# 3dlg-hcvc/minsu3d

Hardware: AMD Instinct MI355X
Metric: scenes/sec (fwd+bwd) PointGroup on ~150k-pt 2cm voxels (higher is better)
Workload: dtype f32; 1 GPU; PointGroup m=16, synthetic ScanNet-shaped scenes (~144k points, ~106k voxels @2cm each), 4 scenes/GPU/step, grouping+ScoreNet branch on, fwd+loss+bwd+Adam; scenes_per_gpu=4, parallelism=dp1, grouping_inputs=GT labels, GT offsets + N(0,4cm) (random-init net groups nothing)

## Files before the change

### include/minsu3d_hip.h

```cpp
#ifndef MINSU3D_HIP_H
#define MINSU3D_HIP_H
#include <stddef.h>
#include <stdint.h>

#ifdef __cplusplus
extern "C" {
#endif

#define MS3D_E_WORKSPACE 10001
#define MS3D_E_UNSUPPORTED 10002
#define MS3D_E_INTERNAL 10003

typedef void *ms3d_stream_t;

const char *ms3d_version(void);

size_t ms3d_ballquery_workspace_bytes(int n);
int ms3d_ballquery_batch_p(int n, int meanActive, float radius, const float *xyz, const uint8_t *batch_idxs,
                           const int *batch_offsets, int n_scenes, int max_scene_points, int *idx,
                           int *start_len, int *n_active , int *capped ,
                           void *workspace, size_t workspace_bytes, ms3d_stream_t stream);

size_t ms3d_bfs_workspace_bytes(int N);
int ms3d_pg_bfs_cluster(const int16_t *semantic_label, const int *ball_query_idxs, long n_edges ,
// ... 310 lines not shown
                                 void *ev_wg_stop, float *ws_wgrad, ms3d_stream_t wgrad_stream, int join,
                                 float *wgrad_slabs, int *wgrad_deferred_nblk, void *wgrad_deferred_launch, int precision,
                                 ms3d_stream_t stream);
int ms3d_spconv_wgrad_is_bf16x3_g(int Vout, int K, int Cin, int Cout, int offset_list, int submanifold);
int ms3d_spconv_backward_weight_g(const float *in, const float *dout, const int *nbr, int Vin, int Vout, int K, int Cin,
                                  int Cout, float *dW, const float *pre_scale, const float *pre_shift, int pre_relu,
                                  float *partial_ws, const int *ol_kt_start, const int *ol_entries, int submanifold,
                                  int precision, ms3d_stream_t stream);
int ms3d_spconv_layer_backward_g(const float *x, const float *dy, const float *wf_buf, const int *nbr_fwd,
                                 const int *nbr_bwd, int Vin, int Vout, int K, int Cin, int Cout, const float *scale,
                                 const float *shift, const float *mean, const float *invstd, int pre_relu, int training,
                                 int need_dx, float *dx, const float *dx_add, float *dgb, float *dW, float *ws,
                                 const int *ol_fwd_kt_start, const int *ol_fwd_entries, const int *pl_bwd_tile_start,
                                 const int *pl_bwd_entries, void *ev_start, void *ev_stop, void *ev_wg_start,
                                 void *ev_wg_stop, float *ws_wgrad, ms3d_stream_t wgrad_stream, int join,
                                 float *wgrad_slabs, int *wgrad_deferred_nblk, void *wgrad_deferred_launch, int precision,
                                 int submanifold, ms3d_stream_t stream);
size_t ms3d_spconv_wgrad_launch_bytes(void);
int ms3d_spconv_wgrad_is_table_walk(int Vout, int K, int Cin, int Cout, int offset_list);
int ms3d_spconv_wgrad_multi(const void *descs, int n_desc, int total_blocks, int variant, ms3d_stream_t stream);
int ms3d_wgrad_reduce_blocks(long n, const float *slabs, const float *dW, int *wide );
int ms3d_wgrad_reduce_multi(const void *descs, int n_desc, int total_blocks, ms3d_stream_t stream);

int ms3d_bn_stats(const float *x, long V, int C, float eps, float momentum, const float *gamma, const float *beta,
                  float *running_mean, float *running_var, float *mean, float *invstd, float *scale, float *shift,
                  float *partial_ws, int partial_rows, ms3d_stream_t stream);
int ms3d_bn_apply(const float *x, long V, int C, const float *scale, const float *shift, int relu, float *y,
                  ms3d_stream_t stream);
int ms3d_reduce_partials(const float *partial, int nparts, int n, float *out, ms3d_stream_t stream);
int ms3d_column_sum(const float *x, long V, int C, float *partial_ws, int partial_rows, float *out2c, ms3d_stream_t stream);
int ms3d_bn_bwd_apply(const float *dz, const float *x, long V, int C, const float *scale, const float *mean,
                      const float *invstd, const float *s1s2, float *dx, ms3d_stream_t stream);
int ms3d_bn_bwd_reduce_apply(const float *partial, int nparts, const float *dz, const float *x, long V, int C,
                             const float *scale, const float *mean, const float *invstd, const float *add, float *dx,
                             float *s1s2, ms3d_stream_t stream);
int ms3d_bn_bwd_apply_add(const float *dz, const float *x, long V, int C, const float *scale, const float *mean,
                          const float *invstd, const float *s1s2, const float *add, float *dx, ms3d_stream_t stream);
int ms3d_bn_bwd_partial(const float *dy, const float *x, long V, int C, const float *scale, const float *shift,
                        const float *mean, const float *invstd, int relu, float *dz, float *partial_ws,
                        int partial_rows, int *nparts_out , ms3d_stream_t stream);

int ms3d_dense_tile_cells(void);
int ms3d_dense_tile_channels(void);
int ms3d_dense_cell_map(const int *coords, int V, const int *origin , int divisor, int B, int X, int Y, int Z,
                        int *cell_row, int *row_cell, int *counts_dev, int *counts , ms3d_stream_t stream);
int ms3d_dense_scatter(const float *F, long n_rows, long ld, const int *cell_row, const int *row_index, int B, int C, int X,
                       int Y, int Z, float *out , ms3d_stream_t stream);
int ms3d_dense_gather(const float *grid, int B, int C, int X, int Y, int Z, const int *cells, long n, float *out,
                      ms3d_stream_t stream);
size_t ms3d_dense_occupancy_workspace_bytes(void);
int ms3d_dense_occupancy(const float *grid, int B, int C, int X, int Y, int Z, unsigned char *keep, int *rank,
                         int *n_kept , void *workspace, size_t workspace_bytes, ms3d_stream_t stream);
int ms3d_dense_cells_emit(const unsigned char *keep, const int *rank, int B, int X, int Y, int Z, int *out_coords,
                          int *out_cells, ms3d_stream_t stream);

int ms3d_proposal_cross_intersection(const int *pair_point, const int *pair_cluster, int S, int P, int *inter ,
                                     ms3d_stream_t stream);
int ms3d_nms_greedy(const int *inter, const int *order, int P, float threshold, unsigned char *suppressed_ws, int *pick,
                    int *n_pick, ms3d_stream_t stream);

int ms3d_elastic_distort(const double *xyz , int N, float *noise, float *noise_tmp, int bx, int by, int bz,
                         double gran, double mag, double *out , ms3d_stream_t stream);

int ms3d_adam_chunk_elems(void);
int ms3d_adam_step(const int *chunks, int n_chunks, void *const *p_ptrs, const void *const *g_ptrs, void *const *m_ptrs,
                   void *const *v_ptrs, const long *sizes, float lr, float beta1, float beta2, float eps,
                   float weight_decay, double bias_correction1, double bias_correction2, ms3d_stream_t stream);
int ms3d_adam_step_multi(const int *chunks, int n_chunks, void *const *p_ptrs, const void *const *g_ptrs,
                         void *const *m_ptrs, void *const *v_ptrs, const long *sizes, const float *coef, float beta1,
                         float beta2, float eps, float weight_decay, ms3d_stream_t stream);

size_t ms3d_scan_i32_workspace_bytes(void);
int ms3d_scan_i32(const int *in, int *out, int n, int *total_out_dev, void *workspace, ms3d_stream_t stream);

int ms3d_point_losses_blocks(long N);
int ms3d_point_losses_forward(const float *scores , const short *labels , const float *pred_offsets ,
                              const float *centre , const float *xyz , const short *instance_ids ,
                              long N, int C, float *d_scores, float *d_norm, float *d_dir, double *partial_ws, float *out5,
                              ms3d_stream_t stream);
int ms3d_point_losses_scale_grads(float *d_scores, long n_scores, float *d_norm, const float *d_dir, long n_off,
                                  const float *out5, const float *g_sem, const float *g_norm, const float *g_dir,
                                  ms3d_stream_t stream);

#ifdef __cplusplus
}
#endif
#endif
```

### minsu3d_amd/_lib.py

```python
import ctypes as C
import os

_HERE = os.path.dirname(os.path.abspath(__file__))
LIB_PATH = os.environ.get("MS3D_LIB") or os.path.join(_HERE, "lib", "libminsu3d_hip.so")
_lib = None


class HipLibraryError(RuntimeError):
    pass


def lib():
    global _lib
    if _lib is None:
        if not os.path.exists(LIB_PATH):
            raise HipLibraryError(
                f"{LIB_PATH} is missing: run `python -c 'import __graft_entry__ as g; g.build()'` "
                "(hipcc --offload-arch=gfx950). There is no CPU fallback in the product path.")
        _lib = C.CDLL(LIB_PATH)
        _lib.ms3d_version.restype = C.c_char_p
        for name in ("ms3d_ballquery_workspace_bytes", "ms3d_bfs_workspace_bytes", "ms3d_hais_workspace_bytes",
                     "ms3d_coord_workspace_bytes", "ms3d_coords_expand_workspace_bytes",
                     "ms3d_coords_union_workspace_bytes", "ms3d_broadcast_reduce_workspace_bytes",
                     "ms3d_chconv_wgrad_ws_floats", "ms3d_kattn_dbias_ws_floats", "ms3d_inorm_workspace_bytes",
                     "ms3d_dense_occupancy_workspace_bytes", "ms3d_kmap_pairs_workspace_bytes",
                     "ms3d_qattn_ws_floats", "ms3d_qattn_backward_ws_floats", "ms3d_vattn_backward_kv_ws_floats"):
            if hasattr(_lib, name):
                getattr(_lib, name).restype = C.c_size_t
        if hasattr(_lib, "ms3d_qattn_chunks"):
            _lib.ms3d_qattn_chunks.restype = C.c_long
    return _lib


E_UNSUPPORTED = 10002


def check(rc, what):
    if rc != 0:
        raise HipLibraryError(f"{what} failed with code {rc}")


def ptr(t):
    if t is None:
        return C.c_void_p(0)
    assert t.is_contiguous(), "tensor must be contiguous"
    return C.c_void_p(t.data_ptr())


_raw_stream = None


def stream_handle():
    global _raw_stream
    import torch
    if _raw_stream is None:
        _raw_stream = getattr(torch._C, "_cuda_getCurrentRawStream", False)
    if _raw_stream:
        return C.c_void_p(_raw_stream(torch._C._cuda_getDevice()))
    return C.c_void_p(torch.cuda.current_stream().cuda_stream)
```

### minsu3d_amd/backend.py

```python
import ctypes as C
import os
import weakref

import numpy as np
import torch

from . import _lib

_BACKEND = None


def get_backend():
    global _BACKEND
    if _BACKEND is None:
        _BACKEND = HipBackend()
    return _BACKEND


def set_backend(b):
    global _BACKEND
    prev = _BACKEND
    _BACKEND = b
    return prev

# ... 212 lines not shown

    def __init__(self):
        self.lib = _lib.lib()
        self.ext = _load_host_ext() if not os.environ.get("MS3D_LIB") else None
        self.ws = _Workspace()
        self.kernel_timer = None
        self.weight_token = 0
        self.matmul_precision_aware = True
        self._prep_table = None

    @staticmethod
    def _dev(t):
        if not t.is_cuda:
            if not torch.cuda.is_available():
                raise _lib.HipLibraryError("HipBackend needs a GPU (got a CPU tensor and no device is present); "
                                           "the product path has no CPU fallback")
            t = t.cuda(non_blocking=True)
        return t.contiguous()

    def ballquery_batch_p(self, coords, batch_idxs, batch_offsets, radius, meanActive, max_scene_points=0):
        coords = self._dev(coords); batch_idxs = self._dev(batch_idxs); batch_offsets = self._dev(batch_offsets)
        n = coords.size(0)
        dev = coords.device
        start_len = torch.zeros((n, 2), dtype=torch.int32, device=dev)
        if n == 0:
            return torch.zeros(0, dtype=torch.int32, device=dev), start_len
        if max_scene_points <= 0:
            max_scene_points = SCENE_BOUNDS.get(batch_offsets)
            if max_scene_points is None:
                max_scene_points = int((batch_offsets[1:] - batch_offsets[:-1]).max().item())
                SCENE_BOUNDS.put(batch_offsets, max_scene_points)
        ws_bytes = self.lib.ms3d_ballquery_workspace_bytes(n)
        ws = self.ws.get("bq", ws_bytes, dev)
        n_active, capped = C.c_int(0), C.c_int(0)
        timer = self.kernel_timer
        ev0 = timer.op_begin() if timer is not None else None
        hint_key = (round(float(radius), 6), int(meanActive))
        hints = self.__dict__.setdefault("_bq_mean_active", {})
        meanActive = max(int(meanActive), hints.get(hint_key, 0))
        while True:
            idx = torch.empty(n * meanActive, dtype=torch.int32, device=dev)
            rc = self.lib.ms3d_ballquery_batch_p(
                n, int(meanActive), C.c_float(radius), _lib.ptr(coords), _lib.ptr(batch_idxs),
                _lib.ptr(batch_offsets), int(batch_offsets.numel() - 1), int(max_scene_points), _lib.ptr(idx),
                _lib.ptr(start_len), C.byref(n_active), C.byref(capped), _lib.ptr(ws), C.c_size_t(ws.numel()),
                _lib.stream_handle())
            _lib.check(rc, "ms3d_ballquery_batch_p")
            if n_active.value <= n * meanActive:
                break
            meanActive = int(n_active.value // n + 1)
            hints[hint_key] = meanActive + meanActive // 8 + 1
        if ev0 is not None:
            timer.op_end("ballquery_batch_p", ev0, n * 20 + n_active.value * (6.64 * 12 + 4))
        GRAPHS.put(start_len, int(capped.value))
        return idx[:n_active.value], start_len

    def _bfs(self, fn_name, args_head, ball_idx, start_len, args_tail):
        hint = int(GRAPHS.get(start_len, -1))
        ball_idx = self._dev(ball_idx); start_len = self._dev(start_len)
        N = start_len.size(0)
        dev = start_len.device
        cluster_idxs = torch.empty((max(N, 1), 2), dtype=torch.int32, device=dev)
        cluster_offsets = torch.empty(N + 1, dtype=torch.int32, device=dev)
        ws_bytes = self.lib.ms3d_bfs_workspace_bytes(N)
        ws = self.ws.get("bfs", ws_bytes, dev)
        counts = (C.c_int * 2)(0, 0)
        args_tail = tuple(hint if a is _HINT else a for a in args_tail)
        timer = self.kernel_timer
        ev0 = timer.op_begin() if timer is not None else None
        rc = getattr(self.lib, fn_name)(*args_head, _lib.ptr(ball_idx), C.c_long(ball_idx.numel()), _lib.ptr(start_len), N,
                                        *args_tail,
                                        _lib.ptr(cluster_idxs), _lib.ptr(cluster_offsets), counts, _lib.ptr(ws),
                                        C.c_size_t(ws.numel()), _lib.stream_handle())
        _lib.check(rc, fn_name)
        if ev0 is not None:
            timer.op_end(fn_name[5:], ev0, ball_idx.numel() * 4 + N * 14 + counts[1] * 8)
        return cluster_idxs[:counts[1]], cluster_offsets[:counts[0] + 1]

    def pg_bfs_cluster(self, semantic_label, ball_query_idxs, start_len, threshold):
        sem = self._dev(semantic_label)
        assert sem.dtype == torch.int16
        return self._bfs("ms3d_pg_bfs_cluster", (_lib.ptr(sem),), ball_query_idxs, start_len, (int(threshold), _HINT))

    def sg_bfs_cluster(self, class_numpoint_mean, ball_query_idxs, start_len, threshold, class_id):
        mean = (C.c_float * len(class_numpoint_mean))(*[float(x) for x in class_numpoint_mean])
        return self._bfs("ms3d_sg_bfs_cluster", (mean,), ball_query_idxs, start_len,
                         (C.c_float(threshold), _HINT, int(class_id)))

    def sg_bfs_cluster_batched(self, group_of_point, thr_per_group, ball_query_idxs, start_len):
        g = self._dev(group_of_point); t = self._dev(thr_per_group)
        assert g.dtype == torch.uint8 and t.dtype == torch.float32
        return self._bfs("ms3d_sg_bfs_cluster_batched", (_lib.ptr(g), _lib.ptr(t)), ball_query_idxs, start_len, (_HINT,))

    def hierarchical_aggregation(self, sem, coord_shift, ball_idx, start_len, batch_idxs, using_set_aggr,
                                 point_num_avg, radius_avg, ignored_label=-1):
        hint = int(GRAPHS.get(start_len, -1))
        sem = self._dev(sem); cs = self._dev(coord_shift); ball_idx = self._dev(ball_idx)
        start_len = self._dev(start_len); batch_idxs = self._dev(batch_idxs)
        assert sem.dtype == torch.int16 and batch_idxs.dtype == torch.uint8
        N, dev, ncls = start_len.size(0), start_len.device, len(point_num_avg)
        pna = (C.c_float * ncls)(*[float(x) for x in point_num_avg])
        ra = (C.c_float * ncls)(*[float(x) for x in radius_avg])
        out_idx = torch.empty((max(2 * N, 1), 2), dtype=torch.int32, device=dev)
        out_off = torch.empty(N + 1, dtype=torch.int32, device=dev)
        self.lib.ms3d_hais_workspace_bytes.restype = C.c_size_t
        ws = self.ws.get("hais", self.lib.ms3d_hais_workspace_bytes(N, ncls), dev)
        counts = (C.c_int * 2)(0, 0)
        timer = self.kernel_timer
        ev0 = timer.op_begin() if timer is not None else None
        _lib.check(self.lib.ms3d_hierarchical_aggregation(
            _lib.ptr(sem), _lib.ptr(cs), _lib.ptr(batch_idxs), _lib.ptr(ball_idx), C.c_long(ball_idx.numel()),
            _lib.ptr(start_len), N, hint, int(bool(using_set_aggr)), pna, ra, ncls, _lib.ptr(out_idx), _lib.ptr(out_off),
            counts, _lib.ptr(ws), C.c_size_t(ws.numel()), _lib.stream_handle()), "ms3d_hierarchical_aggregation")
        if ev0 is not None:
            timer.op_end("hierarchical_aggregation", ev0, ball_idx.numel() * 4 + N * 14 + counts[1] * 8 + N * 12)
        return out_idx[:counts[1]], out_off[:counts[0] + 1]

    def hierarchical_aggregation_parts(self, sem, coord_shift, ball_idx, start_len, batch_idxs, using_set_aggr,
                                       point_num_avg, radius_avg):
        hint = int(GRAPHS.get(start_len, -1))
        sem = self._dev(sem); cs = self._dev(coord_shift); ball_idx = self._dev(ball_idx)
        start_len = self._dev(start_len); batch_idxs = self._dev(batch_idxs)
        assert sem.dtype == torch.int16 and batch_idxs.dtype == torch.uint8
        N, dev, ncls = start_len.size(0), start_len.device, len(point_num_avg)
        pna = (C.c_float * ncls)(*[float(x) for x in point_num_avg])
        ra = (C.c_float * ncls)(*[float(x) for x in radius_avg])
        M = max(N, 1)
        ib = torch.empty((4, M, 2), dtype=torch.int32, device=dev)
        ob = torch.empty((4, M + 1), dtype=torch.int32, device=dev)
        cb = torch.empty((3, M, 5), dtype=torch.float32, device=dev)
        self.lib.ms3d_hais_workspace_bytes.restype = C.c_size_t
        ws = self.ws.get("hais", self.lib.ms3d_hais_workspace_bytes(N, ncls), dev)
        counts = (C.c_int * 8)()
        _lib.check(self.lib.ms3d_hierarchical_aggregation_parts(
            _lib.ptr(sem), _lib.ptr(cs), _lib.ptr(batch_idxs), _lib.ptr(ball_idx), C.c_long(ball_idx.numel()),
            _lib.ptr(start_len), N, hint, int(bool(using_set_aggr)), pna, ra, ncls,
            _lib.ptr(ib[0]), _lib.ptr(ob[0]), _lib.ptr(cb[0]), _lib.ptr(ib[1]), _lib.ptr(ob[1]), _lib.ptr(cb[1]),
            _lib.ptr(ib[2]), _lib.ptr(ob[2]), _lib.ptr(cb[2]), _lib.ptr(ib[3]), _lib.ptr(ob[3]), counts,
            _lib.ptr(ws), C.c_size_t(ws.numel()), _lib.stream_handle()), "ms3d_hierarchical_aggregation_parts")
        nk, rk, npr, _rpost, nf, rf, rp = [counts[i] for i in range(7)]
        out = {"kept": (ib[0, :rk], ob[0, :nk + 1], cb[0, :nk]), "primary": (ib[1, :rp], ob[1, :npr + 1], cb[1, :npr]),
               "fragment": None, "post": None}
        if using_set_aggr:
            out["fragment"] = (ib[2, :rf], ob[2, :nf + 1], cb[2, :nf])
            out["post"] = (ib[3, :rf + rp], ob[3, :npr + 1])
        return out

    def _seg(self, fn_name, inp, offsets):
        inp = self._dev(inp); offsets = self._dev(offsets)
        P, Cc = offsets.numel() - 1, inp.size(1)
        out = torch.zeros((P, Cc), dtype=torch.float32, device=inp.device)
        rc = getattr(self.lib, fn_name)(P, Cc, _lib.ptr(inp), _lib.ptr(offsets), _lib.ptr(out), _lib.stream_handle())
        _lib.check(rc, fn_name)
        return out

    def sec_mean(self, inp, offsets): return self._seg("ms3d_sec_mean", inp, offsets)
    def sec_min(self, inp, offsets): return self._seg("ms3d_sec_min", inp, offsets)
    def sec_max(self, inp, offsets): return self._seg("ms3d_sec_max", inp, offsets)
    def global_avg_pool_fp(self, feats, offsets): return self._seg("ms3d_global_avg_pool_fp", feats, offsets)

    def proposal_voxel_coords(self, clusters_idx, clusters_offset, coords, scale, spatial_shape, rand6):
        ci = self._dev(clusters_idx); off = self._dev(clusters_offset); xyz = self._dev(coords); r6 = self._dev(rand6)
        assert ci.dtype == torch.int64 and ci.is_contiguous() and off.dtype == torch.int32
        assert xyz.dtype == torch.float32 and xyz.is_contiguous() and r6.dtype == torch.float32 and r6.numel() == 6
        S, P, dev = ci.size(0), off.numel() - 1, xyz.device
        out = torch.empty((S, 4), dtype=torch.int32, device=dev)
# ... 120 lines not shown
        prop_idx = self._dev(prop_idx); prop_off = self._dev(prop_off); iou = self._dev(iou)
        P, I = iou.shape
        ml = torch.zeros(prop_idx.shape, dtype=torch.bool, device=prop_idx.device)
        mlm = torch.zeros(prop_idx.shape, dtype=torch.bool, device=prop_idx.device)
        rc = self.lib.ms3d_get_mask_label(I, P, int(ignored_label), C.c_float(iou_thr), _lib.ptr(prop_idx),
                                          _lib.ptr(prop_off), _lib.ptr(self._dev(inst_labels)),
                                          _lib.ptr(self._dev(inst_cls)), _lib.ptr(iou), _lib.ptr(ml), _lib.ptr(mlm),
                                          _lib.stream_handle())
        _lib.check(rc, "ms3d_get_mask_label")
        return ml, mlm


def _f32(t):
    return None if t is None else t.contiguous()


def _p(t):
    return None if t is None else t.data_ptr()


_VP, _I = C.c_void_p, C.c_int
_FAST_ARGTYPES = {
    "ms3d_spconv_layer_forward": [_VP] * 3 + [_I] * 5 + [_VP] * 2 + [_I] + [_VP] * 5 + [_VP] * 2 + [_VP] * 2 + [_VP],
    "ms3d_spconv_layer_backward": [_VP] * 5 + [_I] * 5 + [_VP] * 4 + [_I] * 3 + [_VP] * 5 + [_VP] * 4 + [_VP] * 4 +
                                  [_VP, _VP, _I, _VP, _VP, _VP, _VP],
    "ms3d_spconv_layer_forward_p": [_VP] * 3 + [_I] * 5 + [_VP] * 2 + [_I] + [_VP] * 5 + [_VP] * 2 + [_VP] * 2 + [_I, _VP],
    "ms3d_spconv_layer_backward_p": [_VP] * 5 + [_I] * 5 + [_VP] * 4 + [_I] * 3 + [_VP] * 5 + [_VP] * 4 + [_VP] * 4 +
                                    [_VP, _VP, _I, _VP, _VP, _VP, _I, _VP],
    "ms3d_spconv_layer_backward_g": [_VP] * 5 + [_I] * 5 + [_VP] * 4 + [_I] * 3 + [_VP] * 5 + [_VP] * 4 + [_VP] * 4 +
                                    [_VP, _VP, _I, _VP, _VP, _VP, _I, _I, _VP],
    "ms3d_bn_finalize": [_VP, _I, C.c_long, _I, C.c_float, C.c_float] + [_VP] * 4 + [_VP] * 4 + [_VP],
}


class KernelTimer:

    def __init__(self, lib):
        self.lib = lib
        lib.ms3d_event_create.restype = C.c_void_p
        lib.ms3d_event_elapsed_ms.restype = C.c_float
        self.records = []
        self.sampling = False
        self.steps_sampled = 0
        self._pool = []

    def reserve(self, n_events):
        while len(self._pool) < n_events:
            self._pool.append(C.c_void_p(self.lib.ms3d_event_create()))

    def _event(self):
        return self._pool.pop() if self._pool else C.c_void_p(self.lib.ms3d_event_create())

    def conv(self, kind, K, cin, cout, nbr, rows):
        if not self.sampling:
            return None
        pairs = table_lists(nbr).pair_count()
        ev = (self._event(), self._event())
        self.records.append((("spconv_" + kind, K, cin, cout, rows), ev[0], ev[1],
                             (pairs, (cin + cout) * 4 + 8, K * cin * cout * 4), 2 * cin * cout))
        return ev

    def conv_group(self, kind, layers):
        if not self.sampling or not layers:
            return None
        ev = (self._event(), self._event())
        parts = []
        for K, cin, cout, rows, nbr in layers:
            parts.append((table_lists(nbr).pair_count(), (cin + cout) * 4 + 8, K * cin * cout * 4, 2 * cin * cout))
        K, cin, cout, rows, _ = layers[0]
        self.records.append((("spconv_" + kind, K, cin, cout, rows, len(layers)), ev[0], ev[1], parts, None))
        return ev

    def op_begin(self):
        if not self.sampling:
            return None
        ev = self._event()
        self.lib.ms3d_event_record(ev, _lib.stream_handle())
        return ev

    def op_end(self, name, ev0, nbytes):
        ev1 = self._event()
        self.lib.ms3d_event_record(ev1, _lib.stream_handle())
        self.records.append(((name,), ev0, ev1, float(nbytes), 0))

    def summary(self):
        out = {}
        for key, a, b, nb, fpp in self.records:
            ms = self.lib.ms3d_event_elapsed_ms(a, b)
            self.lib.ms3d_event_destroy(a); self.lib.ms3d_event_destroy(b)
            if ms < 0:
                continue
            flops = 0.0
            if isinstance(nb, list):
                tot = 0.0
                for pairs_t, per_pair, const, fpp_l in nb:
                    pairs = float(pairs_t.item())
                    tot += pairs * per_pair + const
                    flops += pairs * fpp_l
                nb = tot
            elif isinstance(nb, tuple):
                pairs = float(nb[0].item())
                flops = pairs * fpp
                nb = pairs * nb[1] + nb[2]
            g = out.setdefault(key, dict(launches=0, ms=0.0, bytes=0.0, flops=0.0))
            g["launches"] += 1; g["ms"] += ms; g["bytes"] += nb; g["flops"] += flops
        self.records = []
        return out


class WgradQueue:
    _host = _host_np = _dev = _copied = None
    _turn = 0
    RING = 16

    side_mode = False

    def __init__(self, lib, timer=None):
        self.lib = lib
        self.items = []
        self.launches = []
        self.timer = timer

    def add(self, slabs, dW, n, nblk):
        assert int(nblk) * int(n) <= slabs.numel(), "more slabs to reduce than the slab tensor holds"
        self.items.append((slabs, dW, int(n), int(nblk)))

    def add_launch(self, desc, keep, timing=None):
        head = np.frombuffer(desc, dtype=np.int32, count=6)
        self.launches.append((int(head[4]), desc, int(head[1]) * int(head[2]) * int(head[3]), keep, timing))

    def flush(self):
        launches, self.launches = self.launches, []
        items, self.items = self.items, []
        if self.side_mode:
            dev_ = items[0][1].device if items else torch.device("cuda", torch.cuda.current_device())
            main, side = torch.cuda.current_stream(dev_), wgrad_stream(dev_)
            if items:
                with torch.cuda.stream(side):
                    self._flush(launches, items)
            main.wait_stream(side)
            return
        self._flush(launches, items)

    def _flush(self, launches, items):
        if not launches and not items:
            return
        dev = (launches[0][3][0] if launches else items[0][1]).device
        by_variant = {}
        for l in launches:
            by_variant.setdefault(l[0], []).append(l)
        rows = 4 * len(launches) + len(items)
        cls = WgradQueue
        if cls._host is None or cls._host[0].shape[0] < rows or cls._dev[0].device != dev:
            cap = (max(2 * rows, 512) + 3) & ~3
            cls._host = [torch.empty((cap, 4), dtype=torch.int64).pin_memory() for _ in range(self.RING)]
            cls._host_np = [h.numpy().view(np.uint64) for h in cls._host]
            cls._dev = [torch.empty((cap, 4), dtype=torch.int64, device=dev) for _ in range(self.RING)]
            cls._copied = [None] * self.RING
        turn = cls._turn
        cls._turn = (turn + 1) % self.RING
        hn, tdev = cls._host_np[turn], cls._dev[turn]
        if cls._copied[turn] is not None:
            cls._copied[turn].synchronize()
        h32 = hn.view(np.int32).reshape(-1, 32)
        plan, row = [], 0
        for variant, group in by_variant.items():
# ... 1220 lines not shown
```

### minsu3d_amd/model/pointgroup.py

```python
import os

import torch
import torch.nn as nn

from .. import MinkowskiEngine as ME
from ..backend import get_backend, side_stream as _side_stream, worker as _worker
from ..common_ops.functions import common_ops, pointgroup_ops
from .general_model import GeneralModel, clusters_voxelization, get_segmented_scores, scene_offsets
from .module import TinyUnet


class PointGroup(GeneralModel):
    def __init__(self, cfg):
        super().__init__(cfg)
        m = cfg.model.network.m
        self.score_net = TinyUnet(m)
        self.score_branch = nn.Linear(m, 1)
        self.voxelization_rand = None

    def _group(self, xyz, batch_idxs, batch_offsets, sem_fg, object_idxs, mean_active, hook=False):
        net = self.hparams.cfg.model.network.cluster
        idx, start_len = common_ops.ballquery_batch_p(xyz, batch_idxs, batch_offsets, net.cluster_radius, mean_active)
        if hook:
            self._after_ballquery()
        prop_idx, prop_off = pointgroup_ops.pg_bfs_cluster(sem_fg, idx, start_len, net.cluster_npoint_thre)
        prop_idx = prop_idx.long()
        prop_idx[:, 1] = object_idxs[prop_idx[:, 1]]
        return prop_idx, prop_off

    def forward(self, data_dict):
        out = super().forward(data_dict)
        self._queue_point_losses(data_dict, out)
        cfg = self.hparams.cfg
        net = cfg.model.network
        if self.current_epoch <= net.prepare_epochs:
            return out
        sem_pred = data_dict.get("grouping_semantic_preds")
        if sem_pred is None:
            sem_pred = out["semantic_scores"].argmax(1).to(torch.int16)
        grouping_offsets = data_dict.get("grouping_point_offsets")
        if grouping_offsets is None:
            grouping_offsets = out["point_offsets"]
        fg = torch.ones_like(sem_pred, dtype=torch.bool)
        for cls in cfg.data.ignore_classes:
            fg &= sem_pred != (cls - 1)
        object_idxs = torch.nonzero(fg).view(-1)
        batch_idxs = data_dict["vert_batch_ids"][object_idxs]
        batch_offsets = scene_offsets(batch_idxs, len(data_dict["scan_ids"]))
        xyz = data_dict["point_xyz"][object_idxs]
        shifted = (xyz + grouping_offsets[object_idxs]).detach().contiguous()
        sem_fg = sem_pred[object_idxs].contiguous()

        xyz = xyz.contiguous()
        if xyz.is_cuda and os.environ.get("MS3D_GROUP_STREAMS", "1") != "0":
            main = torch.cuda.current_stream()
            side = _side_stream(xyz.device)
            timer = getattr(get_backend(), "kernel_timer", None)
            span0 = timer.op_begin() if timer is not None else None
            side.wait_stream(main)

            def second():
                with torch.cuda.stream(side), torch.no_grad():
                    return self._group(xyz, batch_idxs, batch_offsets, sem_fg, object_idxs, net.cluster.cluster_meanActive)

            pending = _worker().submit(second)
            try:
                p_shift, o_shift = self._group(shifted, batch_idxs, batch_offsets, sem_fg, object_idxs,
                                               net.cluster.cluster_shift_meanActive, hook=True)
            finally:
                p_orig, o_orig = pending.result()
                main.wait_stream(side)
            if span0 is not None:
                timer.op_end("grouping span (both ball queries + both BFS, two streams, one interval)", span0, 0)
            p_orig.record_stream(main)
            o_orig.record_stream(main)
        else:
            p_shift, o_shift = self._group(shifted, batch_idxs, batch_offsets, sem_fg, object_idxs,
                                           net.cluster.cluster_shift_meanActive, hook=True)
            p_orig, o_orig = self._group(xyz, batch_idxs, batch_offsets, sem_fg, object_idxs,
                                         net.cluster.cluster_meanActive)
        p_shift[:, 0] += o_orig.size(0) - 1
        proposals_idx = torch.cat((p_orig, p_shift), dim=0)
        proposals_offset = torch.cat((o_orig, o_shift[1:] + o_orig[-1]))

        self._after_grouping()
        if proposals_offset.numel() <= 1:
            out["proposal_scores"] = (out["point_features"].new_zeros((0, 1)), proposals_idx, proposals_offset)
            return out
        self._early_point_backward(data_dict, out)
        vox, p2v = clusters_voxelization(proposals_idx, proposals_offset, out["point_features"],
                                         data_dict["point_xyz"], net.score_scale, net.score_fullscale, self.device,
                                         rand=self.voxelization_rand, max_dup=2)
        score_feats = ME.gather_rows(self.score_net(vox).features, p2v, max_dup=1)
        pooled = common_ops.roipool(score_feats, proposals_offset)
        out["proposal_scores"] = (self.score_branch(pooled), proposals_idx, proposals_offset)
        return out

    def _loss(self, data_dict, output_dict):
        losses = super()._loss(data_dict, output_dict)
        if "proposal_scores" in output_dict:
            net = self.hparams.cfg.model.network
            scores, proposals_idx, proposals_offset = output_dict["proposal_scores"]
            if proposals_offset.numel() > 1:
                ious = common_ops.get_iou(proposals_idx[:, 1].int().contiguous(), proposals_offset,
                                          data_dict["instance_ids"], data_dict["instance_num_point"])
                target = get_segmented_scores(ious.max(1)[0], net.fg_thresh, net.bg_thresh)
                losses["score_loss"] = nn.functional.binary_cross_entropy_with_logits(scores.view(-1), target)
            else:
                losses["score_loss"] = scores.sum() * 0
        return losses

    def _get_pred_instances(self, scan_id, gt_xyz, proposals_scores, proposals_idx, num_proposals, semantic_scores,
                            num_ignored_classes):
        from .postprocess import pointgroup_instances
        t = self.hparams.cfg.model.network.test
        return pointgroup_instances(scan_id, gt_xyz, proposals_scores, proposals_idx, num_proposals, semantic_scores,
                                    num_ignored_classes, t.TEST_SCORE_THRESH, t.TEST_NPOINT_THRESH, t.TEST_NMS_THRESH)
```

Before: 204.3 scenes/sec.

## Fuse PointGroup grouping inputs, ball query+BFS, and proposal join into native kernels

Adds native HIP entry points that build the foreground grouping inputs (flag, scan, compaction, batch offsets) in one call, run ball query and BFS clustering back-to-back in a single library call with a preallocated neighbour capacity, and join the two proposal sets in one kernel. This is meant to replace many small torch ops, host syncs and per-stage allocations on the grouping path. If the neighbour buffer overflows, the code falls back to the old separate ball-query and BFS path. It adds a sizable new code path and still needs a host readback of the counts.

```diff
diff --git a/include/minsu3d_hip.h b/include/minsu3d_hip.h
--- a/include/minsu3d_hip.h
+++ b/include/minsu3d_hip.h
@@ -416,6 +416,25 @@
                                   const float *out5, const float *g_sem, const float *g_norm, const float *g_dir,
                                   ms3d_stream_t stream);
 
+size_t ms3d_pg_group_inputs_workspace_bytes(long N);
+int ms3d_pg_group_inputs(const int16_t *sem_pred, const int *ignore_ids , int n_ignore,
+                         const uint8_t *vert_batch_ids, const float *point_xyz, const float *offsets, long N, int B,
+                         long long *object_idxs, uint8_t *batch_idxs_fg, float *xyz_fg, float *shifted_fg, int16_t *sem_fg,
+                         int *batch_offsets, int *host2 , void *workspace, size_t workspace_bytes,
+                         ms3d_stream_t stream);
+#define MS3D_E_GROUP_OVERFLOW 10004
+long ms3d_pg_group_idx_capacity(int n, int meanActive);
+long ms3d_pg_group_usable_capacity(int n, long idx_capacity);
+int ms3d_pg_group(int n, long idx_capacity, float radius, const float *xyz, const uint8_t *batch_idxs,
+                  const int *batch_offsets, int n_scenes, int max_scene_points, const int16_t *semantic_label,
+                  int threshold, int *idx, int *start_len, int *cluster_idxs , int *cluster_offsets ,
+                  int *host4 , void *bq_workspace, size_t bq_workspace_bytes, void *bfs_workspace,
+                  size_t bfs_workspace_bytes, void *ev_bq_start, void *ev_bq_stop, void *ev_bfs_start, void *ev_bfs_stop,
+                  ms3d_stream_t stream);
+int ms3d_pg_join_proposals(const int *rows_a, long Sa, const int *off_a, int Ca, const int *rows_b, long Sb,
+                           const int *off_b, int Cb, const long long *object_idxs, long n_obj, long long *proposals_idx,
+                           int *proposals_offset, ms3d_stream_t stream);
+
 #ifdef __cplusplus
 }
 #endif
diff --git a/minsu3d_amd/_lib.py b/minsu3d_amd/_lib.py
--- a/minsu3d_amd/_lib.py
+++ b/minsu3d_amd/_lib.py
@@ -24,15 +24,20 @@
                      "ms3d_coords_union_workspace_bytes", "ms3d_broadcast_reduce_workspace_bytes",
                      "ms3d_chconv_wgrad_ws_floats", "ms3d_kattn_dbias_ws_floats", "ms3d_inorm_workspace_bytes",
                      "ms3d_dense_occupancy_workspace_bytes", "ms3d_kmap_pairs_workspace_bytes",
-                     "ms3d_qattn_ws_floats", "ms3d_qattn_backward_ws_floats", "ms3d_vattn_backward_kv_ws_floats"):
+                     "ms3d_qattn_ws_floats", "ms3d_qattn_backward_ws_floats", "ms3d_vattn_backward_kv_ws_floats",
+                     "ms3d_pg_group_inputs_workspace_bytes"):
             if hasattr(_lib, name):
                 getattr(_lib, name).restype = C.c_size_t
         if hasattr(_lib, "ms3d_qattn_chunks"):
             _lib.ms3d_qattn_chunks.restype = C.c_long
+        for name in ("ms3d_pg_group_idx_capacity", "ms3d_pg_group_usable_capacity"):
+            if hasattr(_lib, name):
+                getattr(_lib, name).restype = C.c_long
     return _lib
 
 
 E_UNSUPPORTED = 10002
+E_GROUP_OVERFLOW = 10004
 
 
 def check(rc, what):
diff --git a/minsu3d_amd/backend.py b/minsu3d_amd/backend.py
--- a/minsu3d_amd/backend.py
+++ b/minsu3d_amd/backend.py
@@ -318,6 +318,90 @@
         assert sem.dtype == torch.int16
         return self._bfs("ms3d_pg_bfs_cluster", (_lib.ptr(sem),), ball_query_idxs, start_len, (int(threshold), _HINT))
 
+    def pg_group_inputs(self, sem_pred, ignore_ids, vert_batch_ids, point_xyz, offsets, n_scenes):
+        N, dev = sem_pred.size(0), sem_pred.device
+        assert sem_pred.dtype == torch.int16 and vert_batch_ids.dtype == torch.uint8
+        assert point_xyz.dtype == torch.float32 and offsets.dtype == torch.float32
+        sem_pred = sem_pred.contiguous(); vert_batch_ids = vert_batch_ids.contiguous()
+        point_xyz = point_xyz.contiguous(); offsets = offsets.contiguous()
+        lib = self.lib
+        ws = self.ws.get("pg_inputs", lib.ms3d_pg_group_inputs_workspace_bytes(C.c_long(N)), dev)
+        object_idxs = torch.empty(N, dtype=torch.int64, device=dev)
+        batch_fg = torch.empty(N, dtype=torch.uint8, device=dev)
+        xyz_fg = torch.empty((N, 3), dtype=torch.float32, device=dev)
+        shifted = torch.empty((N, 3), dtype=torch.float32, device=dev)
+        sem_fg = torch.empty(N, dtype=torch.int16, device=dev)
+        batch_offsets = torch.empty(n_scenes + 1, dtype=torch.int32, device=dev)
+        ids = (C.c_int * max(len(ignore_ids), 1))(*[int(i) for i in ignore_ids])
+        host = (C.c_int * 2)(0, 0)
+        _lib.check(lib.ms3d_pg_group_inputs(
+            _lib.ptr(sem_pred), ids, len(ignore_ids), _lib.ptr(vert_batch_ids), _lib.ptr(point_xyz), _lib.ptr(offsets),
+            C.c_long(N), int(n_scenes), _lib.ptr(object_idxs), _lib.ptr(batch_fg), _lib.ptr(xyz_fg), _lib.ptr(shifted),
+            _lib.ptr(sem_fg), _lib.ptr(batch_offsets), host, _lib.ptr(ws), C.c_size_t(ws.numel()), _lib.stream_handle()),
+            "ms3d_pg_group_inputs")
+        n_fg = host[0]
+        SCENE_BOUNDS.put(batch_offsets, int(host[1]))
+        return object_idxs[:n_fg], batch_fg[:n_fg], xyz_fg[:n_fg], shifted[:n_fg], sem_fg[:n_fg], batch_offsets
+
+    def pg_group(self, coords, batch_idxs, batch_offsets, radius, meanActive, semantic_label, threshold,
+                 idx_capacity=None):
+        n, dev = coords.size(0), coords.device
+        if n == 0:
+            idx, start_len = self.ballquery_batch_p(coords, batch_idxs, batch_offsets, radius, meanActive)
+            return (idx, start_len) + tuple(self.pg_bfs_cluster(semantic_label, idx, start_len, threshold))
+        assert semantic_label.dtype == torch.int16
+        max_scene_points = SCENE_BOUNDS.get(batch_offsets)
+        if max_scene_points is None:
+            max_scene_points = int((batch_offsets[1:] - batch_offsets[:-1]).max().item())
+            SCENE_BOUNDS.put(batch_offsets, max_scene_points)
+        lib = self.lib
+        hint_key = (round(float(radius), 6), int(meanActive))
+        hints = self.__dict__.setdefault("_bq_mean_active", {})
+        mean = max(int(meanActive), hints.get(hint_key, 0))
+        cap = n * mean if idx_capacity is None else int(idx_capacity)
+        bq_ws = self.ws.get("bq", lib.ms3d_ballquery_workspace_bytes(n), dev)
+        bfs_ws = self.ws.get("bfs", lib.ms3d_bfs_workspace_bytes(n), dev)
+        idx = torch.empty(cap, dtype=torch.int32, device=dev)
+        start_len = torch.empty((n, 2), dtype=torch.int32, device=dev)
+        rows = torch.empty((n, 2), dtype=torch.int32, device=dev)
+        offs = torch.empty(n + 1, dtype=torch.int32, device=dev)
+        host = (C.c_int * 4)(0, 0, 0, 0)
+        timer = self.kernel_timer
+        ev = timer.op_events(4) if timer is not None else None
+        evp = [e if e is not None else C.c_void_p(0) for e in (ev or (None,) * 4)]
+        rc = lib.ms3d_pg_group(
+            n, C.c_long(cap), C.c_float(radius), _lib.ptr(coords), _lib.ptr(batch_idxs), _lib.ptr(batch_offsets),
+            int(batch_offsets.numel() - 1), int(max_scene_points), _lib.ptr(semantic_label), int(threshold), _lib.ptr(idx),
+            _lib.ptr(start_len), _lib.ptr(rows), _lib.ptr(offs), host, _lib.ptr(bq_ws), C.c_size_t(bq_ws.numel()),
+            _lib.ptr(bfs_ws), C.c_size_t(bfs_ws.numel()), evp[0], evp[1], evp[2], evp[3], _lib.stream_handle())
+        n_active, capped, n_cluster, n_rows = host[0], host[1], host[2], host[3]
+        if rc == _lib.E_GROUP_OVERFLOW:
+            if ev is not None:
+                timer.op_events_unused(ev)
+            idx, start_len = self.ballquery_batch_p(coords, batch_idxs, batch_offsets, radius, meanActive)
+            return (idx, start_len) + tuple(self.pg_bfs_cluster(semantic_label, idx, start_len, threshold))
+        _lib.check(rc, "ms3d_pg_group")
+        if ev is not None:
+            timer.op_pair("ballquery_batch_p", ev[0], ev[1], n * 20 + n_active * (6.64 * 12 + 4))
+            timer.op_pair("pg_bfs_cluster", ev[2], ev[3], n_active * 4 + n * 14 + n_rows * 8)
+        GRAPHS.put(start_len, int(capped))
+        return idx[:n_active], start_len, rows[:n_rows], offs[:n_cluster + 1]
+
+    def pg_join_proposals(self, rows_a, off_a, rows_b, off_b, object_idxs):
+        dev = off_a.device
+        Sa, Sb, Ca, Cb = rows_a.size(0), rows_b.size(0), off_a.numel() - 1, off_b.numel() - 1
+        assert rows_a.dtype == torch.int32 and rows_b.dtype == torch.int32 and object_idxs.dtype == torch.int64
+        assert off_a.dtype == torch.int32 and off_b.dtype == torch.int32 and Ca >= 0 and Cb >= 0
+        proposals_idx = torch.empty((Sa + Sb, 2), dtype=torch.int64, device=dev)
+        proposals_offset = torch.empty(Ca + Cb + 1, dtype=torch.int32, device=dev)
+        rows_a = rows_a.contiguous(); rows_b = rows_b.contiguous(); off_a = off_a.contiguous(); off_b = off_b.contiguous()
+        object_idxs = object_idxs.contiguous()
+        _lib.check(self.lib.ms3d_pg_join_proposals(
+            _lib.ptr(rows_a), C.c_long(Sa), _lib.ptr(off_a), Ca, _lib.ptr(rows_b), C.c_long(Sb), _lib.ptr(off_b), Cb,
+            _lib.ptr(object_idxs), C.c_long(object_idxs.numel()), _lib.ptr(proposals_idx), _lib.ptr(proposals_offset),
+            _lib.stream_handle()), "ms3d_pg_join_proposals")
+        return proposals_idx, proposals_offset
+
     def sg_bfs_cluster(self, class_numpoint_mean, ball_query_idxs, start_len, threshold, class_id):
         mean = (C.c_float * len(class_numpoint_mean))(*[float(x) for x in class_numpoint_mean])
         return self._bfs("ms3d_sg_bfs_cluster", (mean,), ball_query_idxs, start_len,
@@ -604,6 +688,17 @@
         ev1 = self._event()
         self.lib.ms3d_event_record(ev1, _lib.stream_handle())
         self.records.append(((name,), ev0, ev1, float(nbytes), 0))
+
+    def op_events(self, n):
+        if not self.sampling:
+            return None
+        return [self._event() for _ in range(n)]
+
+    def op_pair(self, name, ev0, ev1, nbytes):
+        self.records.append(((name,), ev0, ev1, float(nbytes), 0))
+
+    def op_events_unused(self, events):
+        self._pool.extend(events)
 
     def summary(self):
         out = {}
diff --git a/minsu3d_amd/csrc/group_pipeline.hip b/minsu3d_amd/csrc/group_pipeline.hip
--- /dev/null
+++ b/minsu3d_amd/csrc/group_pipeline.hip
@@ -0,0 +1,243 @@
+#include <algorithm>
+
+#include "common.h"
+#include "scan.h"
+#include "../../include/minsu3d_hip.h"
+
+int ms3d_bfs_run_internal(int mode, int thr_i, float thr_f, int capped_hint, const int16_t *sem, const int *ball_idx,
+                          long n_edges, const int *start_len, int N, int *cluster_idxs, int *cluster_offsets, int *counts,
+                          void *workspace, size_t workspace_bytes, hipStream_t stream);
+
+namespace {
+
+constexpr int GI_MAX_IGNORE = 16;
+constexpr int GI_MAX_SCENES = 256;
+
+struct IgnoreIds {
+    int n;
+    int id[GI_MAX_IGNORE];
+};
+
+struct GiWorkspace {
+    int *flag;
+    int *counts;
+    int *totals;
+    void *scan_ws;
+};
+
+size_t gi_carve(GiWorkspace &w, long N, void *base)
+{
+    char *p = (char *)base;
+    size_t off = 0;
+    auto take = [&](size_t bytes) {
+        void *r = base ? (void *)(p + off) : nullptr;
+        off += ms3d_align(bytes);
+        return r;
+    };
+    w.flag = (int *)take(sizeof(int) * (size_t)N);
+    w.counts = (int *)take(sizeof(int) * GI_MAX_SCENES);
+    w.totals = (int *)take(sizeof(int) * 2);
+    w.scan_ws = take(ms3d_scan_workspace_bytes());
+    return off;
+}
+
+__device__ __forceinline__ bool is_foreground(int s, const IgnoreIds &ig)
+{
+    bool fg = true;
+    for (int k = 0; k < ig.n; k++) fg &= s != ig.id[k];
+    return fg;
+}
+
+__global__ __launch_bounds__(256) void gi_flag_kernel(int N, int B, IgnoreIds ig, const int16_t *__restrict__ sem,
+                                                      const uint8_t *__restrict__ batch, int *__restrict__ flag,
+                                                      int *__restrict__ counts)
+{
+    __shared__ int s_hist[GI_MAX_SCENES];
+    s_hist[threadIdx.x] = 0;
+    __syncthreads();
+    for (long i = (long)blockIdx.x * 256 + threadIdx.x; i < N; i += (long)gridDim.x * 256) {
+        const bool fg = is_foreground(sem[i], ig);
+        flag[i] = fg ? 1 : 0;
+        if (fg) atomicAdd(&s_hist[batch[i]], 1);
+    }
+    __syncthreads();
+    const int c = s_hist[threadIdx.x];
+    if (c != 0 && (int)threadIdx.x < B) atomicAdd(&counts[threadIdx.x], c);
+}
+
+__global__ __launch_bounds__(256) void gi_compact_kernel(int N, IgnoreIds ig, const int16_t *__restrict__ sem,
+                                                         const uint8_t *__restrict__ batch, const float *__restrict__ xyz,
+                                                         const float *__restrict__ offsets, const int *__restrict__ pos,
+                                                         long long *__restrict__ object_idxs, uint8_t *__restrict__ batch_fg,
+                                                         float *__restrict__ xyz_fg, float *__restrict__ shifted_fg,
+                                                         int16_t *__restrict__ sem_fg)
+{
+    for (long i = (long)blockIdx.x * 256 + threadIdx.x; i < N; i += (long)gridDim.x * 256) {
+        const int16_t s = sem[i];
+        if (!is_foreground(s, ig)) continue;
+        const long o = pos[i];
+        object_idxs[o] = (long long)i;
+        batch_fg[o] = batch[i];
+        sem_fg[o] = s;
+#pragma unroll
+        for (int c = 0; c < 3; c++) {
+            const float x = xyz[i * 3 + c];
+            xyz_fg[o * 3 + c] = x;
+            shifted_fg[o * 3 + c] = __fadd_rn(x, offsets[i * 3 + c]);
+        }
+    }
+}
+
+__global__ void gi_offsets_kernel(int B, const int *__restrict__ counts, int *__restrict__ batch_offsets,
+                                  int *__restrict__ totals)
+{
+    if (blockIdx.x != 0 || threadIdx.x != 0) return;
+    int run = 0, big = 0;
+    for (int b = 0; b < B; b++) {
+        batch_offsets[b] = run;
+        const int c = counts[b];
+        run += c;
+        big = max(big, c);
+    }
+    batch_offsets[B] = run;
+    totals[1] = big;
+}
+
+__global__ __launch_bounds__(256) void join_kernel(const int *__restrict__ rows_a, long Sa, const int *__restrict__ off_a,
+                                                   int Ca, const int *__restrict__ rows_b, long Sb,
+                                                   const int *__restrict__ off_b, int Cb,
+                                                   const long long *__restrict__ object_idxs, long n_obj,
+                                                   long long *__restrict__ out_idx, int *__restrict__ out_off)
+{
+    const long S = Sa + Sb;
+    const long C = (long)Ca + Cb + 1;
+    const long work = S > C ? S : C;
+    for (long t = (long)blockIdx.x * 256 + threadIdx.x; t < work; t += (long)gridDim.x * 256) {
+        if (t < S) {
+            const bool second = t >= Sa;
+            const int *row = second ? rows_b + (t - Sa) * 2 : rows_a + t * 2;
+            const long li = row[1];
+            out_idx[t * 2 + 0] = (long long)row[0] + (second ? Ca : 0);
+            out_idx[t * 2 + 1] = (li >= 0 && li < n_obj) ? object_idxs[li] : -1;
+        }
+        if (t < C) out_off[t] = t <= Ca ? off_a[t] : off_b[t - Ca] + off_a[Ca];
+    }
+}
+
+inline int grid_for(long n) { return (int)std::min<long>(std::max<long>((n + 255) / 256, 1), 256 * 32); }
+
+}
+
+extern "C" {
+
+size_t ms3d_pg_group_inputs_workspace_bytes(long N)
+{
+    if (N < 0 || N > 0x7fffffffL) return 0;
+    GiWorkspace w;
+    return gi_carve(w, N > 0 ? N : 1, nullptr);
+}
+
+int ms3d_pg_group_inputs(const int16_t *sem_pred, const int *ignore_ids, int n_ignore, const uint8_t *vert_batch_ids,
+                         const float *point_xyz, const float *offsets, long N, int B, long long *object_idxs,
+                         uint8_t *batch_idxs_fg, float *xyz_fg, float *shifted_fg, int16_t *sem_fg, int *batch_offsets,
+                         int *host2, void *workspace, size_t workspace_bytes, ms3d_stream_t stream_)
+{
+    hipStream_t stream = (hipStream_t)stream_;
+    if (!host2 || !batch_offsets || N < 0 || N > 0x7fffffffL || B < 1 || B > GI_MAX_SCENES || n_ignore < 0 ||
+        n_ignore > GI_MAX_IGNORE || (n_ignore > 0 && !ignore_ids))
+        return MS3D_E_UNSUPPORTED;
+    host2[0] = host2[1] = 0;
+    if (N == 0) {
+        MS3D_CHECK(hipMemsetAsync(batch_offsets, 0, sizeof(int) * ((size_t)B + 1), stream));
+        return 0;
+    }
+    if (!sem_pred || !vert_batch_ids || !point_xyz || !offsets || !object_idxs || !batch_idxs_fg || !xyz_fg || !shifted_fg ||
+        !sem_fg || !workspace)
+        return MS3D_E_UNSUPPORTED;
+    GiWorkspace w;
+    if (gi_carve(w, N, workspace) > workspace_bytes) return MS3D_E_WORKSPACE;
+    IgnoreIds ig;
+    ig.n = n_ignore;
+    for (int k = 0; k < GI_MAX_IGNORE; k++) ig.id[k] = k < n_ignore ? ignore_ids[k] : 0;
+    const int n = (int)N;
+    MS3D_CHECK(hipMemsetAsync(w.counts, 0, sizeof(int) * GI_MAX_SCENES, stream));
+    gi_flag_kernel<<<grid_for(N), 256, 0, stream>>>(n, B, ig, sem_pred, vert_batch_ids, w.flag, w.counts);
+    MS3D_LAUNCH_CHECK();
+    const int rc = ms3d_exclusive_scan_i32(w.flag, w.flag, n, w.totals, w.scan_ws, stream);
+    if (rc) return rc;
+    gi_compact_kernel<<<grid_for(N), 256, 0, stream>>>(n, ig, sem_pred, vert_batch_ids, point_xyz, offsets, w.flag,
+                                                      object_idxs, batch_idxs_fg, xyz_fg, shifted_fg, sem_fg);
+    MS3D_LAUNCH_CHECK();
+    gi_offsets_kernel<<<1, 64, 0, stream>>>(B, w.counts, batch_offsets, w.totals);
+    MS3D_LAUNCH_CHECK();
+    MS3D_CHECK(hipMemcpyAsync(host2, w.totals, sizeof(int) * 2, hipMemcpyDeviceToHost, stream));
+    MS3D_CHECK(hipStreamSynchronize(stream));
+    return 0;
+}
+
+long ms3d_pg_group_idx_capacity(int n, int meanActive)
+{
+    if (n <= 0 || meanActive <= 0) return 0;
+    return (long)n * (long)meanActive;
+}
+
+long ms3d_pg_group_usable_capacity(int n, long idx_capacity)
+{
+    if (n <= 0 || idx_capacity <= 0) return 0;
+    return idx_capacity / n * n;
+}
+
+int ms3d_pg_group(int n, long idx_capacity, float radius, const float *xyz, const uint8_t *batch_idxs,
+                  const int *batch_offsets, int n_scenes, int max_scene_points, const int16_t *semantic_label,
+                  int threshold, int *idx, int *start_len, int *cluster_idxs, int *cluster_offsets, int *host4,
+                  void *bq_workspace, size_t bq_workspace_bytes, void *bfs_workspace, size_t bfs_workspace_bytes,
+                  void *ev_bq_start, void *ev_bq_stop, void *ev_bfs_start, void *ev_bfs_stop, ms3d_stream_t stream_)
+{
+    hipStream_t stream = (hipStream_t)stream_;
+    if (!host4 || !cluster_offsets || idx_capacity < 0) return MS3D_E_UNSUPPORTED;
+    host4[0] = host4[1] = host4[2] = host4[3] = 0;
+    if (n <= 0) {
+        MS3D_CHECK(hipMemsetAsync(cluster_offsets, 0, sizeof(int), stream));
+        return 0;
+    }
+    const long mean = idx_capacity / n;
+    if (mean > 0x7fffffffL) return MS3D_E_UNSUPPORTED;
+    const long usable = ms3d_pg_group_usable_capacity(n, idx_capacity);
+    if (ev_bq_start) MS3D_CHECK(hipEventRecord((hipEvent_t)ev_bq_start, stream));
+    int n_active = 0, capped = 0;
+    int rc = ms3d_ballquery_batch_p(n, (int)mean, radius, xyz, batch_idxs, batch_offsets, n_scenes, max_scene_points, idx,
+                                    start_len, &n_active, &capped, bq_workspace, bq_workspace_bytes, stream_);
+    if (rc) return rc;
+    if (ev_bq_stop) MS3D_CHECK(hipEventRecord((hipEvent_t)ev_bq_stop, stream));
+    host4[0] = n_active;
+    host4[1] = capped;
+    if ((long)n_active > usable) return MS3D_E_GROUP_OVERFLOW;
+    if (ev_bfs_start) MS3D_CHECK(hipEventRecord((hipEvent_t)ev_bfs_start, stream));
+    int counts[2] = {0, 0};
+    rc = ms3d_bfs_run_internal(0, threshold, 0.f, capped, semantic_label, idx, (long)n_active, start_len, n, cluster_idxs,
+                               cluster_offsets, counts, bfs_workspace, bfs_workspace_bytes, stream);
+    if (rc) return rc;
+    if (ev_bfs_stop) MS3D_CHECK(hipEventRecord((hipEvent_t)ev_bfs_stop, stream));
+    host4[2] = counts[0];
+    host4[3] = counts[1];
+    return 0;
+}
+
+int ms3d_pg_join_proposals(const int *rows_a, long Sa, const int *off_a, int Ca, const int *rows_b, long Sb,
+                           const int *off_b, int Cb, const long long *object_idxs, long n_obj, long long *proposals_idx,
+                           int *proposals_offset, ms3d_stream_t stream_)
+{
+    hipStream_t stream = (hipStream_t)stream_;
+    if (Sa < 0 || Sb < 0 || Ca < 0 || Cb < 0 || n_obj < 0 || !off_a || !off_b || !proposals_offset ||
+        (Sa > 0 && !rows_a) || (Sb > 0 && !rows_b) || (Sa + Sb > 0 && (!proposals_idx || !object_idxs)) ||
+        (long)Ca + Cb + 1 > 0x7fffffffL)
+        return MS3D_E_UNSUPPORTED;
+    const long C = (long)Ca + Cb + 1;
+    join_kernel<<<grid_for(std::max<long>(Sa + Sb, C)), 256, 0, stream>>>(rows_a, Sa, off_a, Ca, rows_b, Sb, off_b, Cb,
+                                                                         object_idxs, n_obj, proposals_idx,
+                                                                         proposals_offset);
+    MS3D_LAUNCH_CHECK();
+    return 0;
+}
+
+}
diff --git a/minsu3d_amd/model/pointgroup.py b/minsu3d_amd/model/pointgroup.py
--- a/minsu3d_amd/model/pointgroup.py
+++ b/minsu3d_amd/model/pointgroup.py
@@ -28,6 +28,61 @@
         prop_idx[:, 1] = object_idxs[prop_idx[:, 1]]
         return prop_idx, prop_off
 
+    def _both_groupings(self, group_shifted, group_orig, device):
+        if device.type == "cuda" and os.environ.get("MS3D_GROUP_STREAMS", "1") != "0":
+            main = torch.cuda.current_stream()
+            side = _side_stream(device)
+            timer = getattr(get_backend(), "kernel_timer", None)
+            span0 = timer.op_begin() if timer is not None else None
+            side.wait_stream(main)
+
+            def second():
+                with torch.cuda.stream(side), torch.no_grad():
+                    return group_orig()
+
+            pending = _worker().submit(second)
+            try:
+                shifted = group_shifted()
+            finally:
+                orig = pending.result()
+                main.wait_stream(side)
+            if span0 is not None:
+                timer.op_end("grouping span (both ball queries + both BFS, two streams, one interval)", span0, 0)
+            for t in orig:
+                t.record_stream(main)
+            return shifted, orig
+        return group_shifted(), group_orig()
+
+    def _group_native(self, be, sem_pred, grouping_offsets, data_dict):
+        cfg = self.hparams.cfg
+        net = cfg.model.network.cluster
+        object_idxs, batch_idxs, xyz, shifted, sem_fg, batch_offsets = be.pg_group_inputs(
+            sem_pred, [cls - 1 for cls in cfg.data.ignore_classes], data_dict["vert_batch_ids"], data_dict["point_xyz"],
+            grouping_offsets.detach(), len(data_dict["scan_ids"]))
+
+        def group(coords, mean_active):
+            return be.pg_group(coords, batch_idxs, batch_offsets, net.cluster_radius, mean_active, sem_fg,
+                               net.cluster_npoint_thre)[2:]
+
+        (r_shift, o_shift), (r_orig, o_orig) = self._both_groupings(
+            lambda: group(shifted, net.cluster_shift_meanActive), lambda: group(xyz, net.cluster_meanActive), xyz.device)
+        return be.pg_join_proposals(r_orig, o_orig, r_shift, o_shift, object_idxs)
+
+    def _proposals(self, data_dict, out, proposals_idx, proposals_offset):
+        net = self.hparams.cfg.model.network
+        self._after_grouping()
+        if proposals_offset.numel() <= 1:
+            out["proposal_scores"] = (out["point_features"].new_zeros((0, 1)), proposals_idx, proposals_offset)
+            return out
+        self._early_point_backward(data_dict, out)
+        vox, p2v = clusters_voxelization(proposals_idx, proposals_offset, out["point_features"],
+                                         data_dict["point_xyz"], net.score_scale, net.score_fullscale, self.device,
+                                         rand=self.voxelization_rand, max_dup=2)
+        score_feats = ME.gather_rows(self.score_net(vox).features, p2v, max_dup=1)
+        pooled = common_ops.roipool(score_feats, proposals_offset)
+        out["proposal_scores"] = (self.score_branch(pooled), proposals_idx, proposals_offset)
+        return out
+
     def forward(self, data_dict):
         out = super().forward(data_dict)
         self._queue_point_losses(data_dict, out)
@@ -41,6 +96,13 @@
         grouping_offsets = data_dict.get("grouping_point_offsets")
         if grouping_offsets is None:
             grouping_offsets = out["point_offsets"]
+        be = get_backend()
+        if (sem_pred.is_cuda and os.environ.get("MS3D_GROUP_NATIVE", "1") != "0" and hasattr(be, "pg_group")
+                and "_after_ballquery_fn" not in self.__dict__
+                and sem_pred.dtype == torch.int16 and data_dict["vert_batch_ids"].dtype == torch.uint8
+                and data_dict["point_xyz"].dtype == torch.float32 and grouping_offsets.dtype == torch.float32
+                and len(data_dict["scan_ids"]) <= 256 and len(cfg.data.ignore_classes) <= 16):
+            return self._proposals(data_dict, out, *self._group_native(be, sem_pred, grouping_offsets, data_dict))
         fg = torch.ones_like(sem_pred, dtype=torch.bool)
         for cls in cfg.data.ignore_classes:
             fg &= sem_pred != (cls - 1)
@@ -52,49 +114,15 @@
         sem_fg = sem_pred[object_idxs].contiguous()
 
         xyz = xyz.contiguous()
-        if xyz.is_cuda and os.environ.get("MS3D_GROUP_STREAMS", "1") != "0":
-            main = torch.cuda.current_stream()
-            side = _side_stream(xyz.device)
-            timer = getattr(get_backend(), "kernel_timer", None)
-            span0 = timer.op_begin() if timer is not None else None
-            side.wait_stream(main)
-
-            def second():
-                with torch.cuda.stream(side), torch.no_grad():
-                    return self._group(xyz, batch_idxs, batch_offsets, sem_fg, object_idxs, net.cluster.cluster_meanActive)
-
-            pending = _worker().submit(second)
-            try:
-                p_shift, o_shift = self._group(shifted, batch_idxs, batch_offsets, sem_fg, object_idxs,
-                                               net.cluster.cluster_shift_meanActive, hook=True)
-            finally:
-                p_orig, o_orig = pending.result()
-                main.wait_stream(side)
-            if span0 is not None:
-                timer.op_end("grouping span (both ball queries + both BFS, two streams, one interval)", span0, 0)
-            p_orig.record_stream(main)
-            o_orig.record_stream(main)
-        else:
-            p_shift, o_shift = self._group(shifted, batch_idxs, batch_offsets, sem_fg, object_idxs,
-                                           net.cluster.cluster_shift_meanActive, hook=True)
-            p_orig, o_orig = self._group(xyz, batch_idxs, batch_offsets, sem_fg, object_idxs,
-                                         net.cluster.cluster_meanActive)
+        (p_shift, o_shift), (p_orig, o_orig) = self._both_groupings(
+            lambda: self._group(shifted, batch_idxs, batch_offsets, sem_fg, object_idxs, net.cluster.cluster_shift_meanActive,
+                                hook=True),
+            lambda: self._group(xyz, batch_idxs, batch_offsets, sem_fg, object_idxs, net.cluster.cluster_meanActive),
+            xyz.device)
         p_shift[:, 0] += o_orig.size(0) - 1
         proposals_idx = torch.cat((p_orig, p_shift), dim=0)
         proposals_offset = torch.cat((o_orig, o_shift[1:] + o_orig[-1]))
-
-        self._after_grouping()
-        if proposals_offset.numel() <= 1:
-            out["proposal_scores"] = (out["point_features"].new_zeros((0, 1)), proposals_idx, proposals_offset)
-            return out
-        self._early_point_backward(data_dict, out)
-        vox, p2v = clusters_voxelization(proposals_idx, proposals_offset, out["point_features"],
-                                         data_dict["point_xyz"], net.score_scale, net.score_fullscale, self.device,
-                                         rand=self.voxelization_rand, max_dup=2)
-        score_feats = ME.gather_rows(self.score_net(vox).features, p2v, max_dup=1)
-        pooled = common_ops.roipool(score_feats, proposals_offset)
-        out["proposal_scores"] = (self.score_branch(pooled), proposals_idx, proposals_offset)
-        return out
+        return self._proposals(data_dict, out, proposals_idx, proposals_offset)
 
     def _loss(self, data_dict, output_dict):
         losses = super()._loss(data_dict, output_dict)
```

New measurement: 201.0 scenes/sec. -1.6%, worse.
